# EspressoSystems/Push-CDN

Hardware: NVIDIA H100
Metric: broadcast fan-out egress GB/s (1 KiB x 2^20 subscribers per GPU, 1 topic); msgs/s and % of HBM peak alongside (higher is better)
Workload: dtype u8

## Files before the change

### push-cdn_b200/csrc/engine.cu

```cuda
#include "engine_internal.h"

namespace pcdn_detail {
thread_local std::string g_err;
int fail(int code, const std::string& msg) { g_err = msg; return code; }
}

namespace {

int flush_journal(pcdn_engine* e) {
  HostTables& t = *e->tables;
  if (!e->has_device) { t.clear_dirty(); return 0; }
  const Geometry& g = e->geo;
  bool any = !t.dirty_sub.empty() || !t.dirty_brk.empty() || !t.dirty_owner.empty() || !t.dirty_slots.empty() ||
             !t.dirty_keys.empty();
  if (!any) return 0;
  const uint32_t Ws = e->shard_W(), W = g.W;
  const bool full_keys = t.dirty_keys.size() > (size_t)g.max_keys / 16 + 64;
  const bool full_sub = t.dirty_sub.size() > t.sub.size() / 16 + 64;
  const bool full_slots = t.dirty_slots.size() > t.cuckoo.size() / 16 + 64;
  e->h_slot.clear(); e->h_kslot.clear(); e->h_kbytes.clear();
  if (!full_slots) for (uint32_t i : t.dirty_slots) e->h_slot.push_back(UpdSlot{i, t.cuckoo[i]});
  if (!full_keys) for (uint32_t k : t.dirty_keys) {
    e->h_kslot.push_back(k);
    size_t at = e->h_kbytes.size();
// ... 118 lines not shown
    for (int k = 0; k < 2; k++) {
      const int pv = sh.prev_slot[k];
      if (pv < 0 || pv == (int)si) continue;
      const ShardSlot& o = sh.slots[pv];
      if (cudaEventQuery(o.ev_done) != cudaSuccess) { cudaGetLastError(); continue; }
      const BatchStats& ps_ = *o.h_stats;
      sh.fat_only = ps_.status == 0 && ps_.n_cm == 0 && ps_.n_fat_tiles > 0 && ps_.bytes_out <= kOverlapMaxBytes;
      break;
    }
  }
  const bool fat_overlap = s.in.n_bcast > 0 && sh.fat_only;
  sh.prev_slot[1] = sh.prev_slot[0];
  sh.prev_slot[0] = (int)si;
  cudaStream_t st = sh.stream, ps = (!dp && (direct_only || fat_overlap)) ? sh.pack_stream : sh.stream, cs = sh.copy_stream;
  const bool has_direct = n_direct > 0;
  if (wait_ingest) CUDA_TRY(cudaStreamWaitEvent(st, s.ev_ingest, 0));
  s.timed = e->timing;
  s.polled = false;
  s.n_msg_errors = 0;
  if (!retry && ++s.w.stamp == 0) s.w.stamp = 1;
  if (!retry && sh.dev.pool && (s.w.stamp & 0x3FFFFFFFu) == 0) {
    s.w.stamp++;
    CUDA_TRY(cudaMemsetAsync(s.w.lb_state, 0, ((size_t)sh.dev.N / 256 + 1) * 8, st));
  }
  s.w.pool_unblock = retry ? 1u : 0u;
  s.w.batch_id = retry ? e->slots[si].batch_id : e->next_batch_id;
  const bool fused = dp && sh.dev.N <= kSmallCtrlConns && s.in.n_msgs <= kSmallCtrlMsgs &&
                     (uint64_t)s.in.n_bcast * sh.dev.nblk <= kSmallCtrlItems;
  s.spans_mapped = dp && (sh.dev.N <= 8192 || (s.in.n_bcast == 0 && s.in.n_msgs <= 4096));
  if (sh.dev.pool && !fused) s.spans_mapped = false;
  s.w.spans = s.spans_mapped ? s.d_spans_map : s.d_spans_dev;
  s.w.overflow = s.spans_mapped ? s.d_ovf_map : s.d_ovf_dev;
  const bool zero_in_kernel = fused && !devparse && !retry;
  if (s.timed) CUDA_TRY(cudaEventRecord(s.ev[0], st));
  if (retry) {
    launch_pool_retry_begin(sh.dev, s.w, st);
  } else {
    if (!zero_in_kernel) launch_batch_begin(sh.dev, s.w, s.in, has_direct, st);
    if (devparse) launch_parse(sh.dev, s.w, s.in, st);
    if (has_direct && !fused) launch_direct(sh.dev, s.w, s.in, n_direct, st);
  }
  if (s.timed) CUDA_TRY(cudaEventRecord(s.ev[1], st));
  if (fused) {
    launch_ctrl_small(sh.dev, s.w, s.in, has_direct, zero_in_kernel, s.d_stats_pub, retry, st);
    if (s.timed) { CUDA_TRY(cudaEventRecord(s.ev[2], st)); CUDA_TRY(cudaEventRecord(s.ev[3], st)); }
  } else {
    if (!retry) launch_match(sh.dev, s.w, s.in, st);
    if (s.timed) CUDA_TRY(cudaEventRecord(s.ev[2], st));
    if (!retry) launch_plan(sh.dev, s.w, s.in, st);
    launch_offsets(sh.dev, s.w, s.in, has_direct, sh.n_sms, st);
    if (s.timed) CUDA_TRY(cudaEventRecord(s.ev[3], st));
  }
  if (!s.spans_mapped) {
    CUDA_TRY(cudaEventRecord(s.ev_ctrl, st));
    CUDA_TRY(cudaStreamWaitEvent(cs, s.ev_ctrl, 0));
    CUDA_TRY(cudaMemcpyAsync(s.h_early, s.w.stats, sizeof(BatchStats), cudaMemcpyDeviceToHost, cs));
    CUDA_TRY(cudaEventRecord(s.ev_early, cs));
    if (ps != st) CUDA_TRY(cudaStreamWaitEvent(ps, s.ev_ctrl, 0));
  }
  if (s.timed) CUDA_TRY(cudaEventRecord(s.ev[4], ps));
  uint32_t pack_variant = e->cfg.pack_variant;
  if (!((pack_variant >> 8) & 15u)) pack_variant |= (fat_overlap ? 3u : 4u) << 8;
  launch_pack(sh.dev, s.w, s.in, n_direct, pack_variant, sh.n_sms, ps);
  if (s.timed) CUDA_TRY(cudaEventRecord(s.ev[5], ps));
  CUDA_TRY(cudaGetLastError());
  if (!fused) CUDA_TRY(cudaMemcpyAsync(s.h_stats, s.w.stats, sizeof(BatchStats), cudaMemcpyDeviceToHost, ps));
  CUDA_TRY(cudaEventRecord(s.ev_done, ps));
  return 0;
}

int launch_pipeline(pcdn_engine* e, uint32_t si, bool wait_ingest) {
  Slot& s = e->slots[si];
  for (Shard& sh : e->shards) {
    int rc = launch_shard_pipeline(e, sh, si, s.n_direct, s.devparse, wait_ingest);
    if (rc) return rc;
  }
  s.state = SLOT_INFLIGHT;
  s.t_launch = std::chrono::steady_clock::now();
  s.batch_id = e->next_batch_id++;
  s.counted = false;
  e->inflight.push_back(s.batch_id);
  e->open_slot = -1;
  e->stats.batches++;
  e->stats.msgs += s.n_msgs;
  return 0;
}

struct IngestRegion { const void* src; size_t dst_off; size_t bytes; bool host = false; };
int ingest_batch(pcdn_engine* e, uint32_t si, const IngestRegion* regs, int nregs, bool arena_in_place, bool wait_submit) {
  const size_t all_hi = regs[nregs - 1].dst_off + regs[nregs - 1].bytes;
  if (e->ingest == PCDN_INGEST_HOST) {
    for (Shard& sh : e->shards) {
      DeviceGuard dg(sh.device);
      ShardSlot& ss = sh.slots[si];
      CUDA_TRY(cudaStreamWaitEvent(sh.ingest_stream, ss.ev_done, 0));
      if (wait_submit) CUDA_TRY(cudaStreamWaitEvent(sh.ingest_stream, e->shards[0].ev_submit, 0));
      for (int r = 0; r < nregs; r++) {
        const IngestRegion& g = regs[r];
        if (!g.bytes || (sh.gindex == 0 && r == 0 && arena_in_place)) continue;
// ... 385 lines not shown
  CUDA_TRY(cudaMemsetAsync(d.sub, 0, (size_t)g.T * Ws * 4, sh.stream));
  CUDA_TRY(cudaMemsetAsync(d.brk, 0, (size_t)Ws * 4, sh.stream));
  CUDA_TRY(cudaMemsetAsync(d.owner_conn, 0xFF, (size_t)g.max_owners * 4, sh.stream));
  CUDA_TRY(cudaMemsetAsync(d.cuckoo, 0, (size_t)g.nbuckets * 4 * sizeof(CuckooEntry), sh.stream));
  CUDA_TRY(cudaMemsetAsync(d.keys, 0, (size_t)g.max_keys * g.key_stride, sh.stream));
  CUDA_TRY(cudaMemsetAsync(d.ptail, 0, (size_t)Ns * 4, sh.stream));
  CUDA_TRY(cudaMemsetAsync(d.used, 0, (size_t)Ns * 4, sh.stream));

  const uint32_t M = c.max_batch_msgs, MB = c.max_batch_bcast;
  const size_t cap_fat = (size_t)c.max_batch_deliveries;
  const size_t cap_thin = std::min<size_t>(c.max_batch_deliveries, (size_t)M * (kFatMin - 1));
  sh.slots.resize(c.batch_slots);
  for (ShardSlot& s : sh.slots) {
    DEV_ALLOC(s.d_arena, e->arena_cap);
    Work& w = s.w;
    DEV_ALLOC(w.B, (size_t)MB * Ws);
    DEV_ALLOC(w.wpre, (size_t)MB * Ws);
    DEV_ALLOC(w.cnt, (size_t)MB * d.nblk);
    DEV_ALLOC(w.base, (size_t)MB * d.nblk);
    DEV_ALLOC(w.done, MB);
    CUDA_TRY(cudaMemsetAsync(w.done, 0, (size_t)MB * 4, sh.stream));
    DEV_ALLOC(w.D, M);
    DEV_ALLOC(w.dconn, M);
    DEV_ALLOC(w.eb_fat, (size_t)M + 1);
    DEV_ALLOC(w.eb_thin, (size_t)M + 1);
    DEV_ALLOC(w.tbase, (size_t)M + 1);
    DEV_ALLOC(w.scan_tmp, 4 * ((size_t)M / 256 + 2));
    DEV_ALLOC(w.cls, M);
    DEV_ALLOC(w.cm_rank, (size_t)M + 1);
    DEV_ALLOC(w.cm_list, MB);
    DEV_ALLOC(w.jidx, M);
    DEV_ALLOC(w.efat, cap_fat);
    DEV_ALLOC(w.ecm, cap_fat);
    DEV_ALLOC(w.ethin, cap_thin);
    w.cap_fat = (uint32_t)std::min<size_t>(cap_fat, 0xFFFFFFFFu);
    w.cap_thin = (uint32_t)std::min<size_t>(cap_thin, 0xFFFFFFFFu);
    DEV_ALLOC(w.dcount, (size_t)Ns + 2);
    DEV_ALLOC(w.dloc, (size_t)Ns + 2);
    DEV_ALLOC(w.dtile, (size_t)Ns / 1024 + 3);
    DEV_ALLOC(w.dlist, M);
    DEV_ALLOC(w.hot_list, (size_t)M / kHotMin + 2);
    DEV_ALLOC(w.hot_bitmap, (size_t)kHotCtas * ((size_t)M / 32 + 1));
    DEV_ALLOC(w.scan_done, 1);
    CUDA_TRY(cudaMemsetAsync(w.scan_done, 0, 4, sh.stream));
    DEV_ALLOC(w.edir, M);
    DEV_ALLOC(w.dstart, (size_t)Ns + 1);
    DEV_ALLOC(w.dend, (size_t)Ns + 1);
    DEV_ALLOC(w.dstamp, (size_t)Ns + 1);
    CUDA_TRY(cudaMemsetAsync(w.dstamp, 0, ((size_t)Ns + 1) * 4, sh.stream));
    w.stamp = 0;
    DEV_ALLOC(w.batch_units, Ns);
    if (d.pool) {
      DEV_ALLOC(w.cbase, Ns);
      DEV_ALLOC(w.lb_state, (size_t)Ns / 256 + 1);
      DEV_ALLOC(w.lb_tot, (size_t)Ns / 256 + 1);
      CUDA_TRY(cudaMemsetAsync(w.lb_state, 0, ((size_t)Ns / 256 + 1) * 8, sh.stream));
    }
    w.pool_unblock = 0;
    const size_t span_entries = (size_t)2 * Ns * (d.span_runs ? 3 : 2) / 2;
    DEV_ALLOC(s.d_spans_dev, span_entries);
    DEV_ALLOC(s.d_ovf_dev, Ns);
    if (sh.direct_publish) {
      PIN_ALLOC_MAPPED(s.h_spans, s.d_spans_map, span_entries);
      PIN_ALLOC_MAPPED(s.h_overflow, s.d_ovf_map, (size_t)Ns);
    } else {
      PIN_ALLOC(s.h_spans, span_entries);
      PIN_ALLOC(s.h_overflow, g.shard_max_conns);
    }
    w.spans = s.d_spans_dev; w.overflow = s.d_ovf_dev;
    DEV_ALLOC(w.msg_status, M);
    PIN_ALLOC(s.h_msg_status, M);
    DEV_ALLOC(w.stats, 1);
    if (sh.direct_publish) PIN_ALLOC_MAPPED(s.h_stats, s.d_stats_pub, 1);
    else PIN_ALLOC(s.h_stats, 1);
    PIN_ALLOC(s.h_early, 1);
    CUDA_TRY(cudaEventCreateWithFlags(&s.ev_done, cudaEventDisableTiming));
    CUDA_TRY(cudaEventCreateWithFlags(&s.ev_ctrl, cudaEventDisableTiming));
    CUDA_TRY(cudaEventCreateWithFlags(&s.ev_early, cudaEventDisableTiming));
    CUDA_TRY(cudaEventCreateWithFlags(&s.ev_ingest, cudaEventDisableTiming));
    for (auto& ev : s.ev) CUDA_TRY(cudaEventCreate(&ev));
  }
  CUDA_TRY(cudaStreamSynchronize(sh.stream));
  return 0;
}

int init_nccl(pcdn_engine* e) {
  const char* why = "";
  e->nccl = nccl_api(&why);
  if (!e->nccl) return fail(PCDN_ENODEV, std::string("PCDN_INGEST_NCCL needs libnccl.so.2: ") + why);
  NcclUniqueId id;
  if (e->cfg.nccl_unique_id) std::memcpy(&id, e->cfg.nccl_unique_id, sizeof(id));
  else NCCL_TRY(e->nccl, e->nccl->GetUniqueId(&id));
  NCCL_TRY(e->nccl, e->nccl->GroupStart());
  for (Shard& sh : e->shards) {
    cudaSetDevice(sh.device);
    int rc = e->nccl->CommInitRank(&sh.comm, (int)e->world_shards, id, (int)sh.gindex);
    if (rc) { e->nccl->GroupEnd(); return fail(PCDN_ECUDA, std::string("ncclCommInitRank: ") + e->nccl->GetErrorString(rc)); }
  }
  NCCL_TRY(e->nccl, e->nccl->GroupEnd());
  for (Shard& sh : e->shards) {
    int n = 0;
    if (e->nccl->CommCount && e->nccl->CommCount(sh.comm, &n) == 0) sh.nccl_ranks = n;
  }
  return 0;
}

int init_device(pcdn_engine* e) {
// ... 1042 lines not shown
```

### push-cdn_b200/csrc/kernels.cu

```cuda
#include "kernels.cuh"

#include <atomic>

#include "frame_parse_core.h"

namespace pcdn {

std::atomic<unsigned long long> g_kernel_launches{0};
#define PCDN_COUNT_LAUNCH (void)g_kernel_launches.fetch_add(1, std::memory_order_relaxed)

unsigned long long kernel_launches() { return g_kernel_launches.load(std::memory_order_relaxed); }
void count_kernel_launch() { PCDN_COUNT_LAUNCH; }

__device__ __forceinline__ uint32_t lane_id() { return threadIdx.x & 31; }

__device__ __forceinline__ uint32_t warp_incl_scan(uint32_t v) {
  const uint32_t lane = lane_id();
#pragma unroll
  for (int o = 1; o < 32; o <<= 1) {
    uint32_t n = __shfl_up_sync(0xffffffffu, v, o);
    if (lane >= (uint32_t)o) v += n;
  }
  return v;
}
// ... 345 lines not shown
      const uint32_t q = (c - c_lo) >> 5, k = c & 31u;
      const uint32_t bit = event_bit(s, b, m, wd0 + q, k, e, e1);
#pragma unroll
      for (int x = 0; x < NW; x++)
        if ((uint32_t)x == q) v[x] = (v[x] & ~(1u << k)) | (bit << k);
    }
    while (e1 < ne && b.events[e1].conn == c) e1++;
    e = e1;
  }
}

__device__ __forceinline__ uint32_t match_word(const DevState& s, const BatchIn& b, uint32_t m, uint32_t wd) {
  const uint32_t toff = b.aux_off[m], tn = b.aux_len[m];
  const uint32_t fl = b.flags[m];
  uint32_t word = 0;
  if (fl & MSGF_TOPICS_U8) {
    const uint8_t* tb = b.arena + toff;
    for (uint32_t i = 0; i < tn; i++) {
      if ((fl & MSGF_PRUNE) && !topic_kept(tb, i, s.n_valid_topics)) continue;
      const uint32_t t = tb[i];
      if (t < s.T) word |= s.sub[(size_t)t * s.W + wd];
    }
  } else {
    for (uint32_t i = 0; i < tn; i++) {
      const uint32_t t = b.topics[toff + i];
      if (t < s.T) word |= s.sub[(size_t)t * s.W + wd];
    }
  }
  if (b.n_events) apply_events<1>(s, b, m, wd, &word);
  if (fl & MSGF_USERS_ONLY) word &= ~s.brk[wd];
  return word;
}
template <bool EVENTS>
__global__ void __launch_bounds__(256) k_match(DevState s, BatchIn b, Work w) {
  const uint32_t j = blockIdx.y, lane = lane_id();
  const uint32_t blk = blockIdx.x * 8 + (threadIdx.x >> 5);
  if (blk >= s.nblk) return;
  const uint32_t m = b.bcast_index[j];
  const uint32_t w0 = blk * kBlockWords + lane * 8;
  const uint32_t toff = b.aux_off[m], tn = b.aux_len[m], fl = b.flags[m];
  uint4 lo = make_uint4(0, 0, 0, 0), hi = make_uint4(0, 0, 0, 0);
  auto or_row = [&](uint32_t t) {
    if (t >= s.T) return;
    const uint4* row = reinterpret_cast<const uint4*>(s.sub + (size_t)t * s.W + w0);
    const uint4 a = row[0], c = row[1];
    lo.x |= a.x; lo.y |= a.y; lo.z |= a.z; lo.w |= a.w;
    hi.x |= c.x; hi.y |= c.y; hi.z |= c.z; hi.w |= c.w;
  };
  if (fl & MSGF_TOPICS_U8) {
    const uint8_t* tb = b.arena + toff;
    for (uint32_t i = 0; i < tn; i++) {
      if ((fl & MSGF_PRUNE) && !topic_kept(tb, i, s.n_valid_topics)) continue;
      or_row(tb[i]);
    }
  } else {
    for (uint32_t i = 0; i < tn; i++) or_row(b.topics[toff + i]);
  }
  if (EVENTS) {
    uint32_t v[8] = {lo.x, lo.y, lo.z, lo.w, hi.x, hi.y, hi.z, hi.w};
    apply_events<8>(s, b, m, w0, v);
    lo = make_uint4(v[0], v[1], v[2], v[3]); hi = make_uint4(v[4], v[5], v[6], v[7]);
  }
  if (fl & MSGF_USERS_ONLY) {
    const uint4* br = reinterpret_cast<const uint4*>(s.brk + w0);
    const uint4 a = br[0], c = br[1];
    lo.x &= ~a.x; lo.y &= ~a.y; lo.z &= ~a.z; lo.w &= ~a.w;
    hi.x &= ~c.x; hi.y &= ~c.y; hi.z &= ~c.z; hi.w &= ~c.w;
  }
  const uint32_t p0 = __popc(lo.x), p1 = p0 + __popc(lo.y), p2 = p1 + __popc(lo.z), p3 = p2 + __popc(lo.w);
  const uint32_t p4 = p3 + __popc(hi.x), p5 = p4 + __popc(hi.y), p6 = p5 + __popc(hi.z), p7 = p6 + __popc(hi.w);
  const uint32_t incl = warp_incl_scan(p7), ex = incl - p7;
  uint32_t last = 0;
  if (lane == 31) {
    w.cnt[(size_t)j * s.nblk + blk] = incl;
    __threadfence();
    last = atomicAdd(&w.done[j], 1u) == s.nblk - 1 ? 1u : 0u;
  }
  uint4* Bo = reinterpret_cast<uint4*>(w.B + (size_t)j * s.W + w0);
  Bo[0] = lo; Bo[1] = hi;
  uint4 pre;
  pre.x = ex | ((ex + p0) << 16); pre.y = (ex + p1) | ((ex + p2) << 16);
  pre.z = (ex + p3) | ((ex + p4) << 16); pre.w = (ex + p5) | ((ex + p6) << 16);
  *reinterpret_cast<uint4*>(w.wpre + (size_t)j * s.W + w0) = pre;
  if (__shfl_sync(0xffffffffu, last, 31)) {
    __threadfence();
    uint32_t carry = 0;
    for (uint32_t bb = 0; bb < s.nblk; bb += 32) {
      const uint32_t i = bb + lane;
      const uint32_t v = i < s.nblk ? __ldcg(w.cnt + (size_t)j * s.nblk + i) : 0;
      const uint32_t in = warp_incl_scan(v);
      if (i < s.nblk) w.base[(size_t)j * s.nblk + i] = carry + in - v;
      carry += __shfl_sync(0xffffffffu, in, 31);
    }
    if (lane == 0) { w.D[m] = carry; w.jidx[m] = j; w.done[j] = 0; }
  }
}
void launch_match(const DevState& s, const Work& w, const BatchIn& b, cudaStream_t st) {
  if (!b.n_bcast) return;
  dim3 grid((s.nblk + 7) / 8, b.n_bcast);
  if (b.n_events) PCDN_COUNT_LAUNCH, k_match<true><<<grid, 256, 0, st>>>(s, b, w);
  else PCDN_COUNT_LAUNCH, k_match<false><<<grid, 256, 0, st>>>(s, b, w);
}

__device__ __forceinline__ uint32_t frame_vec_bytes(uint32_t raw_len) { return (4u + raw_len + 15u) & ~15u; }
__device__ __forceinline__ uint32_t frame_units(uint32_t raw_len) { return (4u + raw_len + kUnit - 1u) / kUnit; }
__device__ __forceinline__ uint32_t rec_units(const DevState& s, uint32_t raw_len) {
  return s.shared_payload ? 1u : frame_units(raw_len);
}
__device__ __forceinline__ uint32_t tile_recipients(uint32_t frame_bytes) {
  const uint32_t chunk = min(frame_bytes, kChunkBytes);
  return max(32u, min(kTileRecipients, kFatTileBytes / chunk));
}

__device__ __forceinline__ void plan_classify(const DevState& s, const BatchIn& b, uint32_t m, uint32_t d, uint32_t* cls_out,
                                              uint32_t* tiles_out) {
  uint32_t cls = CLS_THIN, tiles = 0;
  if (d >= kFatMin) {
    const uint32_t len = b.raw_len[m];
    const bool dense = !s.shared_payload && ((uint64_t)d << kCmDenseShift) >= s.N && b.kind[m] == 4;
    if (dense && frame_units(len) * kUnit <= kCmMaxBytes) {
      cls = CLS_CM;
    } else {
      cls = CLS_FAT;
      const uint32_t nch = (frame_vec_bytes(len) + kChunkBytes - 1) / kChunkBytes;
      const uint32_t tr = tile_recipients(frame_vec_bytes(len));
      tiles = nch * ((d + tr - 1) / tr);
    }
  }
  *cls_out = cls; *tiles_out = tiles;
}

__global__ void __launch_bounds__(256) k_plan_a(DevState s, BatchIn b, Work w, uint32_t nblk) {
  __shared__ uint32_t sm[9];
  const uint32_t m = blockIdx.x * 256 + threadIdx.x;
// ... 148 lines not shown
  __shared__ uint32_t sm[NW + 1];
  __shared__ unsigned long long red[2][NW];
  __shared__ uint32_t span_base;
  if (w.stats->status) return;
  const uint32_t wd = c >> 5, lane = c & 31, lt = (1u << lane) - 1u;
  const uint32_t R = s.pool ? 0x7FFFFFFFu : s.ring_units;
  ConnCursor k;
  k.pt = s.pool ? 0u : s.ptail[c]; k.us = s.pool ? 0u : s.used[c]; k.bu = 0;
  k.s1_off = 0; k.s1_units = 0; k.s1_rec = 0; k.s2_units = 0; k.s2_rec = 0; k.ovf = 0; k.in2 = 0; k.bytes = 0;
  uint32_t dp = 0, de = 0;
  if (HAS_DIRECT) {
    if (SPARSE_BOUNDS) {
      if (w.dstamp[c] == w.stamp) { dp = w.dstart[c]; de = w.dend[c]; }
    } else {
      dp = dseg_start(w, c); de = dseg_start(w, c + 1);
      if (de - dp >= 2 && de - dp <= kHotMin) {
        for (uint32_t i = dp + 1; i < de; i++) {
          const uint32_t x = w.dlist[i];
          uint32_t j = i;
          while (j > dp && w.dlist[j - 1] > x) { w.dlist[j] = w.dlist[j - 1]; j--; }
          w.dlist[j] = x;
        }
      }
    }
  }
  const uint32_t* dmsg = w.dlist;

  auto emit_direct = [&](uint32_t m) {
    const uint32_t len = b.raw_len[m];
    const uint32_t off = alloc_record(k, rec_units(s, len), R, len);
    w.edir[m] = make_uint2(c, off);
  };

  __shared__ uint32_t m_mb[32], m_len[32], m_eb[32], m_slot[32], m_cls[32];
  for (uint32_t j0 = 0; j0 < b.n_bcast; j0 += 32) {
    const uint32_t nj = min(32u, b.n_bcast - j0);
    __syncthreads();
    if (threadIdx.x < nj) {
      const uint32_t m = b.bcast_index[j0 + threadIdx.x];
      const uint32_t cl = w.cls[m];
      m_mb[threadIdx.x] = m;
      m_len[threadIdx.x] = b.raw_len[m];
      m_cls[threadIdx.x] = cl;
      m_eb[threadIdx.x] = cl != CLS_THIN ? w.eb_fat[m] : w.eb_thin[m];
      m_slot[threadIdx.x] = b.slot_off16[m];
    }
    uint32_t Bw = 0, pre = 0;
    if (lane < nj) {
      const size_t at = (size_t)(j0 + lane) * s.W + wd;
      Bw = w.B[at];
      pre = w.base[(size_t)(j0 + lane) * s.nblk + (wd / kBlockWords)] + w.wpre[at];
    }
    __syncthreads();
    uint32_t hits = __ballot_sync(0xffffffffu, Bw != 0);
    while (hits) {
      const int i = __ffs(hits) - 1;
      hits &= hits - 1;
      const uint32_t word = __shfl_sync(0xffffffffu, Bw, i), p = __shfl_sync(0xffffffffu, pre, i);
      const uint32_t mb = m_mb[i];
      if (HAS_DIRECT) while (dp < de && dmsg[dp] < mb) { emit_direct(dmsg[dp]); dp++; }
      if ((word >> lane) & 1u) {
        const uint32_t rank = p + __popc(word & lt), len = m_len[i];
        const uint32_t off = alloc_record(k, rec_units(s, len), R, len);
        const uint32_t cl = m_cls[i];
        if (cl == CLS_CM) w.ecm[m_eb[i] + rank] = off;
        else if (cl == CLS_FAT) w.efat[m_eb[i] + rank] = make_uint2(c, off);
        else w.ethin[m_eb[i] + rank] = make_uint4(c, off, m_slot[i], len);
      }
    }
  }
  if (HAS_DIRECT) while (dp < de) { emit_direct(dmsg[dp]); dp++; }

  if (s.pool) {
    __shared__ uint32_t cta_prefix;
    uint32_t ctot;
    const uint32_t cex = cta_excl_scan<NW>(k.bu, &ctot, sm);
    if (LOOKBACK) {
      if (threadIdx.x < 32) {
        const uint32_t pre = pool_lookback(w, vb, ctot);
        if (threadIdx.x == 0) {
          cta_prefix = pre;
          if (vb == nvb - 1) pool_allocate(s, w, (unsigned long long)pre + ctot);
        }
      }
    } else if (threadIdx.x == 0) {
      cta_prefix = 0;
      w.lb_tot[vb] = ctot;
    }
    __syncthreads();
    k.s1_off = cta_prefix + cex;
    w.cbase[c] = k.s1_off;
  } else {
    s.ptail[c] = k.pt;
    s.used[c] = k.us;
  }
  w.batch_units[c] = k.bu;

  const uint32_t nsp = (k.s1_rec ? 1u : 0u) + (k.s2_rec ? 1u : 0u);
  uint32_t tot, ex;
// ... 176 lines not shown
    if (valid) {
      w.eb_fat[m] = e0; w.eb_thin[m] = e1; w.tbase[m] = e2; w.cm_rank[m] = e3; w.cls[m] = (uint8_t)cls;
      if (cls == CLS_CM) w.cm_list[e3] = m;
    }
    if (tid == 0) {
      w.stats->n_fat_entries = t0; w.stats->n_thin_entries = t1; w.stats->n_fat_tiles = t2; w.stats->tile_cursor = 0;
      w.stats->n_cm = t3; w.stats->cm_cursor = 0;
      if (t0 > w.cap_fat || t1 > w.cap_thin) w.stats->status = 1;
      const uint32_t n = b.n_msgs;
      w.eb_fat[n] = t0; w.eb_thin[n] = t1; w.tbase[n] = t2; w.cm_rank[n] = t3;
    }
  }
  cluster_sync_all();

  for (uint32_t c0 = 0; c0 < s.N; c0 += 8192)
    offsets_body<HAS_DIRECT, 1024, true, true>(s, b, w, s.N, c0 + rank * 1024 + tid, c0 / 1024 + rank, s.N / 1024);

  if (publish) {
    cluster_sync_all();
    if (rank == 0 && tid < sizeof(BatchStats) / 4)
      reinterpret_cast<uint32_t*>(publish)[tid] = __ldcg(reinterpret_cast<const uint32_t*>(w.stats) + tid);
  }
}
void launch_ctrl_small(const DevState& s, const Work& w, const BatchIn& b, bool has_direct, bool zero_stats,
                       BatchStats* publish, bool offsets_only, cudaStream_t st) {
  if (has_direct) PCDN_COUNT_LAUNCH, k_ctrl_small<true><<<8, 1024, 0, st>>>(s, b, w, zero_stats ? 1 : 0, publish, offsets_only ? 1 : 0);
  else PCDN_COUNT_LAUNCH, k_ctrl_small<false><<<8, 1024, 0, st>>>(s, b, w, zero_stats ? 1 : 0, publish, offsets_only ? 1 : 0);
}

__global__ void k_pool_retry_begin(BatchStats* bs) {
  bs->status = 0;
  bs->n_deliveries = 0; bs->bytes_out = 0;
  bs->n_spans = 0; bs->n_runs = 0; bs->n_overflow = 0;
  bs->tile_cursor = 0; bs->cm_cursor = 0;
}
void launch_pool_retry_begin(const DevState& s, const Work& w, cudaStream_t st) {
  cudaMemsetAsync(w.lb_state, 0, ((size_t)s.N / 256 + 1) * 8, st);
  PCDN_COUNT_LAUNCH, k_pool_retry_begin<<<1, 1, 0, st>>>(w.stats);
}

__device__ __forceinline__ uint8_t* conn_out(const DevState& s, const Work& w, uint32_t conn, uint32_t pool_base) {
  return s.pool ? s.rings + ((size_t)pool_base + w.cbase[conn]) * kUnit : s.rings + (size_t)conn * s.ring_bytes;
}

__device__ __forceinline__ void pack_fat_phase(const DevState& s, const BatchIn& b, const Work& w, uint8_t* buf,
                                               uint64_t* barp) {
  uint64_t& bar = *barp;
  __shared__ uint32_t t_info[8];
  const uint32_t tid = threadIdx.x;
  const uint32_t ntiles = w.stats->n_fat_tiles;
  if (ntiles == 0) return;
  const uint32_t pool_base = w.stats->pool_base;
  uint32_t phase = 0;
  uint32_t staged_m = 0xFFFFFFFFu, staged_k = 0xFFFFFFFFu;

  for (;;) {
    if (tid == 0) {
      const uint32_t t = atomicAdd(&w.stats->tile_cursor, 1u);
      t_info[0] = t;
      if (t < ntiles) {
        uint32_t lo = 0, hi = b.n_msgs;
        while (hi - lo > 1) { uint32_t mid = (lo + hi) >> 1; if (w.tbase[mid] <= t) lo = mid; else hi = mid; }
        const uint32_t m = lo, ltile = t - w.tbase[m], d = w.D[m];
        const uint32_t fb = frame_vec_bytes(b.raw_len[m]);
        const uint32_t tr = tile_recipients(fb);
        const uint32_t ngrp = (d + tr - 1) / tr;
        const uint32_t ch = ltile / ngrp, grp = ltile % ngrp;
// ... 37 lines not shown
  bulk_wait_read0();
}

__device__ __forceinline__ void pack_cm_phase(const DevState& s, const BatchIn& b, const Work& w, uint8_t* buf,
                                              uint64_t* barp) {
  uint64_t& bar = *barp;
  __shared__ uint32_t g_m[kCmGroup], g_j[kCmGroup], g_soff[kCmGroup], g_units[kCmGroup], g_eb[kCmGroup];
  __shared__ uint32_t t_info[4];
  const uint32_t tid = threadIdx.x, lane = tid & 31, warp = tid >> 5;
  if (w.stats->status) return;
  const uint32_t ncm = w.stats->n_cm;
  if (ncm == 0) return;
  const uint32_t pool_base = w.stats->pool_base;
  const uint32_t ngroups = (ncm + kCmGroup - 1) / kCmGroup;
  const uint32_t tpg = s.W / kCmTileWords;
  const uint32_t ntiles = ngroups * tpg;
  uint32_t phase = 0;
  uint32_t staged_g = 0xFFFFFFFFu;

  for (;;) {
    if (tid == 0) {
      const uint32_t t = atomicAdd(&w.stats->cm_cursor, 1u);
      t_info[0] = t;
      if (t < ntiles) {
        const uint32_t g = t / tpg;
        const uint32_t gcount = min(kCmGroup, ncm - g * kCmGroup);
        t_info[1] = g; t_info[2] = gcount;
        t_info[3] = g != staged_g ? 1u : 0u;
        staged_g = g;
      }
    }
    __syncthreads();
    if (t_info[0] >= ntiles) break;
    const uint32_t gcount = t_info[2];
    if (t_info[3]) {
      bulk_wait_read0();
      __syncthreads();
      if (tid == 0) {
        const uint32_t g = t_info[1];
        uint32_t soff = 0, total = 0;
        for (uint32_t i = 0; i < gcount; i++) {
          const uint32_t m = w.cm_list[g * kCmGroup + i];
          const uint32_t len = b.raw_len[m];
          g_m[i] = m; g_j[i] = w.jidx[m]; g_soff[i] = soff; g_units[i] = frame_units(len); g_eb[i] = w.eb_fat[m];
          soff += frame_units(len) * kUnit;
          total += frame_vec_bytes(len);
        }
        mbar_arrive_expect_tx(&bar, total);
        for (uint32_t i = 0; i < gcount; i++)
          bulk_g2s(buf + g_soff[i], b.arena + (size_t)b.slot_off16[g_m[i]] * 16, frame_vec_bytes(b.raw_len[g_m[i]]), &bar);
      }
      __syncthreads();
      mbar_wait(&bar, phase);
      phase ^= 1;
      if (tid < gcount) {
        *reinterpret_cast<uint32_t*>(buf + g_soff[tid]) = bswap32(b.raw_len[g_m[tid]]);
        fence_proxy_async_smem();
      }
      __syncthreads();
    }
    const uint32_t wt = t_info[0] % tpg;
    for (uint32_t wi = warp; wi < kCmTileWords; wi += 8) {
      const uint32_t wd = wt * kCmTileWords + wi;
      const uint32_t myword = lane < gcount ? w.B[(size_t)g_j[lane] * s.W + wd] : 0u;
      const uint32_t any = __reduce_or_sync(0xffffffffu, myword);
      if (!any) continue;
      uint32_t offs[kCmGroup];
#pragma unroll
      for (int i = 0; i < (int)kCmGroup; i++) {
        const uint32_t wordi = __shfl_sync(0xffffffffu, myword, i);
        offs[i] = kOffInvalid;
        if ((uint32_t)i < gcount && ((wordi >> lane) & 1u)) {
          const uint32_t j = g_j[i];
          const uint32_t idx = g_eb[i] + w.base[(size_t)j * s.nblk + wd / kBlockWords] + w.wpre[(size_t)j * s.W + wd] +
                               __popc(wordi & ((1u << lane) - 1u));
          offs[i] = w.ecm[idx];
        }
      }
      uint8_t* ring = conn_out(s, w, wd * 32 + lane, pool_base);
      uint32_t run_o = kOffInvalid, run_units = 0, run_s = 0;
#pragma unroll
      for (int i = 0; i < (int)kCmGroup; i++) {
        const uint32_t o = offs[i];
        if (o != kOffInvalid && run_o != kOffInvalid && o == run_o + run_units) {
          run_units += g_units[i];
        } else {
          if (run_o != kOffInvalid) bulk_s2g(ring + (size_t)run_o * kUnit, buf + run_s, run_units * kUnit);
          run_o = o; run_s = g_soff[i]; run_units = (o != kOffInvalid) ? g_units[i] : 0;
        }
      }
      if (run_o != kOffInvalid) bulk_s2g(ring + (size_t)run_o * kUnit, buf + run_s, run_units * kUnit);
    }
    bulk_commit();
    __syncthreads();
  }
  bulk_wait_read0();
}

__device__ __forceinline__ void copy_record(const uint4* __restrict__ src, uint4* __restrict__ dst, uint32_t raw_len, uint32_t lane) {
  const uint32_t nvec = (4u + raw_len + 15u) >> 4;
  const uint32_t hdr = bswap32(raw_len);
  for (uint32_t v = lane; v < nvec; v += 128) {
    uint4 x0, x1, x2, x3;
    const bool p1 = v + 32 < nvec, p2 = v + 64 < nvec, p3 = v + 96 < nvec;
    x0 = ld_nc16(src + v);
    if (p1) x1 = ld_nc16(src + v + 32);
    if (p2) x2 = ld_nc16(src + v + 64);
    if (p3) x3 = ld_nc16(src + v + 96);
    if (v == 0) x0.x = hdr;
// ... 4 lines not shown
  }
}
__device__ __forceinline__ void pack_thin_phase(const DevState& s, const BatchIn& b, const Work& w) {
  const uint32_t n = w.stats->n_thin_entries;
  const uint32_t pool_base = w.stats->pool_base;
  const uint32_t lane = lane_id();
  const uint32_t gw = (blockIdx.x * blockDim.x + threadIdx.x) >> 5, nw = (gridDim.x * blockDim.x) >> 5;
  for (uint32_t e = gw; e < n; e += nw) {
    const uint4 ent = w.ethin[e];
    if (ent.y == kOffInvalid) continue;
    copy_record(reinterpret_cast<const uint4*>(b.arena + (size_t)ent.z * 16),
                reinterpret_cast<uint4*>(conn_out(s, w, ent.x, pool_base) + (size_t)ent.y * kUnit), ent.w, lane);
  }
}
__device__ __forceinline__ void pack_direct_phase(const DevState& s, const BatchIn& b, const Work& w) {
  const uint32_t n = b.n_msgs;
  const uint32_t pool_base = w.stats->pool_base;
  const uint32_t lane = lane_id();
  const uint32_t gw = (blockIdx.x * blockDim.x + threadIdx.x) >> 5, nw = (gridDim.x * blockDim.x) >> 5;
  uint2 ent = make_uint2(0, kOffInvalid);
  uint32_t so = 0, len = 0;
  if (gw < n) { ent = w.edir[gw]; so = b.slot_off16[gw]; len = b.raw_len[gw]; }
  for (uint32_t m = gw; m < n; m += nw) {
    const uint2 cur = ent;
    const uint32_t cso = so, clen = len;
    const uint32_t nx = m + nw;
    if (nx < n) { ent = w.edir[nx]; so = b.slot_off16[nx]; len = b.raw_len[nx]; }
    if (cur.y == kOffInvalid) continue;
    copy_record(reinterpret_cast<const uint4*>(b.arena + (size_t)cso * 16),
                reinterpret_cast<uint4*>(conn_out(s, w, cur.x, pool_base) + (size_t)cur.y * kUnit), clen, lane);
  }
}

__global__ void __launch_bounds__(256) k_pack(DevState s, BatchIn b, Work w, int do_direct) {
  __shared__ __align__(128) uint8_t buf[kCmGroup * kCmMaxBytes];
  __shared__ __align__(8) uint64_t bars[2];
  if (w.stats->status) return;
  if (threadIdx.x == 0) {
    mbar_init(&bars[0], 1);
    mbar_init(&bars[1], 1);
    asm volatile("fence.mbarrier_init.release.cluster;" ::: "memory");
  }
  __syncthreads();
  pack_cm_phase(s, b, w, buf, &bars[0]);
  __syncthreads();
  pack_fat_phase(s, b, w, buf, &bars[1]);
  pack_thin_phase(s, b, w);
  if (do_direct) pack_direct_phase(s, b, w);
}
__global__ void __launch_bounds__(256, 8) k_pack_direct(DevState s, BatchIn b, Work w) {
  if (w.stats->status) return;
  pack_direct_phase(s, b, w);
}

__device__ __forceinline__ void st_ref_record(uint8_t* dst, uint32_t raw_len, uint32_t slot_off16, unsigned long long batch_id) {
  const unsigned long long off = (unsigned long long)slot_off16 * 16u + 4u;
  st_stream16(dst, make_uint4(0xFFFFFFFFu, bswap32(raw_len), (uint32_t)off, (uint32_t)(off >> 32)));
  st_stream16(dst + 16, make_uint4((uint32_t)batch_id, (uint32_t)(batch_id >> 32), 0u, 0u));
}
__global__ void __launch_bounds__(256) k_pack_ref(DevState s, BatchIn b, Work w, int do_direct) {
  if (w.stats->status) return;
  const uint32_t nfat = w.stats->n_fat_entries, nthin = w.stats->n_thin_entries;
  const uint64_t nft = (uint64_t)nfat + nthin, total = nft + (do_direct ? b.n_msgs : 0u);
  const uint32_t pool_base = w.stats->pool_base;
  const unsigned long long bid = w.batch_id;
  const uint64_t stride = (uint64_t)gridDim.x * blockDim.x;
  for (uint64_t i = (uint64_t)blockIdx.x * blockDim.x + threadIdx.x; i < total; i += stride) {
    uint32_t conn, off, m = 0, slot = 0, len = 0;
    bool thin = false;
    if (i < nfat) {
      const uint32_t e = (uint32_t)i;
      uint32_t lo = 0, hi = b.n_msgs;
      while (hi - lo > 1) { const uint32_t mid = (lo + hi) >> 1; if (w.eb_fat[mid] <= e) lo = mid; else hi = mid; }
      const uint2 ent = w.efat[e];
      conn = ent.x; off = ent.y; m = lo;
    } else if (i < nft) {
      const uint4 ent = w.ethin[i - nfat];
      conn = ent.x; off = ent.y; slot = ent.z; len = ent.w; thin = true;
    } else {
      m = (uint32_t)(i - nft);
      const uint2 ent = w.edir[m];
      conn = ent.x; off = ent.y;
    }
    if (off == kOffInvalid) continue;
    if (!thin) { slot = b.slot_off16[m]; len = b.raw_len[m]; }
    st_ref_record(conn_out(s, w, conn, pool_base) + (size_t)off * kUnit, len, slot, bid);
  }
}

void launch_pack(const DevState& s, const Work& w, const BatchIn& b, uint32_t n_direct, uint32_t pack_variant, int n_sms, cudaStream_t st) {
  if (s.shared_payload) {
    if (b.n_bcast || n_direct) PCDN_COUNT_LAUNCH, k_pack_ref<<<(uint32_t)n_sms * 8, 256, 0, st>>>(s, b, w, n_direct ? 1 : 0);
    return;
  }
  const bool direct_separate = n_direct >= kThinSeparateMin;
  const uint32_t ctas_per_sm = ((pack_variant >> 8) & 15u) ? ((pack_variant >> 8) & 15u) : 3;
  const uint32_t grid = (uint32_t)n_sms * ctas_per_sm;
  const int do_direct = (n_direct && !direct_separate) ? 1 : 0;
  if (b.n_bcast || do_direct)
    PCDN_COUNT_LAUNCH, k_pack<<<grid, 256, 0, st>>>(s, b, w, do_direct);
  const uint32_t dctas = ((pack_variant >> 12) & 15u) ? ((pack_variant >> 12) & 15u) : 8u;
  if (direct_separate) PCDN_COUNT_LAUNCH, k_pack_direct<<<(uint32_t)n_sms * dctas, 256, 0, st>>>(s, b, w);
}

__global__ void __launch_bounds__(256) k_release(DevState s, const uint32_t* __restrict__ batch_units,
                                                 const BatchStats* __restrict__ stats) {
  if (stats->status) return;
  const uint32_t i = blockIdx.x * blockDim.x + threadIdx.x;
  if (i * 4 < s.N) {
    const uint4 u = reinterpret_cast<const uint4*>(batch_units)[i];
    if (u.x | u.y | u.z | u.w) {
      uint4* p = reinterpret_cast<uint4*>(s.used) + i;
      uint4 v = *p;
      v.x -= u.x; v.y -= u.y; v.z -= u.z; v.w -= u.w;
      *p = v;
    }
  }
}
__global__ void k_pool_release(PoolState* p, const BatchStats* __restrict__ stats) {
  if (stats->status) return;
  p->used -= stats->pool_units + stats->pool_skip;
  p->tail = stats->pool_base + stats->pool_units;
  if (p->used == 0) { p->head = 0; p->tail = 0; }
}
__global__ void k_pool_init(PoolState* p) { p->head = 0; p->tail = 0; p->used = 0; p->blocked = 0; }
void launch_pool_init(const DevState& s, cudaStream_t st) {
  if (s.pool) PCDN_COUNT_LAUNCH, k_pool_init<<<1, 1, 0, st>>>(s.pool_state);
}
void launch_release(const DevState& s, const uint32_t* batch_units, const BatchStats* stats, cudaStream_t st) {
  if (s.pool) { PCDN_COUNT_LAUNCH, k_pool_release<<<1, 1, 0, st>>>(s.pool_state, stats); return; }
  PCDN_COUNT_LAUNCH, k_release<<<(s.N / 4 + 255) / 256, 256, 0, st>>>(s, batch_units, stats);
}

}
```

### push-cdn_b200/csrc/kernels.cuh

```cuda
#pragma once
#include <cuda_runtime.h>
#include <stdint.h>

#include "hash.h"

namespace pcdn {

constexpr uint32_t kUnit = 32;
constexpr uint32_t kOffInvalid = 0xFFFFFFFFu;
constexpr uint32_t kConnNone = 0xFFFFFFFFu;
constexpr uint32_t kFatMin = 32;
constexpr uint32_t kChunkBytes = 16384;
constexpr uint32_t kTileRecipients = 1024;
constexpr uint32_t kFatTileBytes = 131072;
constexpr uint32_t kBlockWords = 256;
constexpr uint32_t kCmGroup = 8;
constexpr uint32_t kCmMaxBytes = 4096;
constexpr uint32_t kSmallCtrlConns = 65536;
constexpr uint32_t kSmallCtrlMsgs = 256;
constexpr uint32_t kSmallCtrlItems = 256;
constexpr uint32_t kThinSeparateMin = 2048;
constexpr uint32_t kHotMin = 32;
constexpr uint32_t kHotCtas = 32;
constexpr uint32_t kCmTileWords = 16;
constexpr uint32_t kCmDenseShift = 4;
enum : uint8_t { CLS_THIN = 0, CLS_FAT = 1, CLS_CM = 2 };
enum : uint8_t {
  MSGF_USERS_ONLY = 1,
  MSGF_DEVPARSE = 2,
  MSGF_TOPICS_U8 = 4,
  MSGF_PRUNE = 8
};
constexpr int8_t kErrParse = -7, kErrPrune = -8;

struct DevState {
  uint32_t* sub;
  uint32_t* brk;
  uint32_t* owner_conn;
  CuckooEntry* cuckoo;
  uint8_t* keys;
  uint32_t* ptail;
  uint32_t* used;
// ... 26 lines not shown
  uint32_t n_msgs, n_bcast;
  const uint8_t* arena;
  const uint8_t* kind;
  const uint8_t* flags;
  const uint32_t* slot_off16;
  const uint32_t* raw_len;
  const uint32_t* aux_off;
  const uint32_t* aux_len;
  const uint16_t* topics;
  const uint32_t* bcast_index;
  uint32_t n_events;
  const SubEvent* events;
  const uint16_t* ev_topics;
};

struct BatchStats {
  unsigned long long n_deliveries;
  unsigned long long bytes_out;
  uint32_t n_spans;
  uint32_t n_overflow;
  uint32_t n_direct_dropped;
  uint32_t status;
  uint32_t n_fat_entries;
  uint32_t n_thin_entries;
  uint32_t n_fat_tiles;
  uint32_t tile_cursor;
  uint32_t n_cm;
  uint32_t cm_cursor;
  uint32_t n_hot;
  uint32_t n_runs;
  uint32_t pool_base;
  uint32_t pool_units;
  uint32_t pool_skip;
  uint32_t reserved;
};

struct PoolState { uint32_t head, tail, used, blocked; };

struct Span { uint32_t conn, ring_off, len, n_records; };
struct SpanRun { uint32_t conn0, n_conns, ring_off, len, n_records, off_stride; };

struct Work {
  uint32_t* B;
  uint16_t* wpre;
  uint32_t* cnt;
  uint32_t* base;
  uint32_t* done;
  uint32_t* D;
  uint32_t* dconn;
  uint32_t* eb_fat;
  uint32_t* eb_thin;
  uint32_t* tbase;
  uint32_t* scan_tmp;
  uint8_t* cls;
  uint32_t* cm_rank;
  uint32_t* cm_list;
  uint32_t* jidx;
  uint2* efat;
  uint32_t* ecm;
  uint4* ethin;
  uint32_t cap_fat, cap_thin;
  uint32_t* dcount;
  uint32_t* dloc;
  uint32_t* dtile;
  uint32_t* dlist;
  uint32_t* hot_list;
  uint32_t* hot_bitmap;
  uint32_t* scan_done;
  uint2* edir;
  uint32_t* dstart;
  uint32_t* dend;
  uint32_t* dstamp;
  uint32_t stamp;
  uint32_t* cbase;
  unsigned long long* lb_state;
  uint32_t* lb_tot;
  uint32_t pool_unblock;
  unsigned long long batch_id;
  uint32_t* batch_units;
  Span* spans;
  uint32_t* overflow;
  int8_t* msg_status;
  BatchStats* stats;
};

struct Upd32 { uint32_t arr, idx, val; };
struct UpdSlot { uint32_t slot; CuckooEntry e; };

void launch_apply_updates(const DevState& s, const Upd32* u32, uint32_t n32, const UpdSlot* us,
                          uint32_t nslot, const uint32_t* key_slots, const uint8_t* key_bytes,
                          uint32_t nkeys, cudaStream_t st);
void launch_batch_begin(const DevState& s, const Work& w, const BatchIn& b, bool has_direct, cudaStream_t st);
void launch_parse(const DevState& s, const Work& w, const BatchIn& b, cudaStream_t st);
void launch_direct(const DevState& s, const Work& w, const BatchIn& b, uint32_t n_direct, cudaStream_t st);
void launch_match(const DevState& s, const Work& w, const BatchIn& b, cudaStream_t st);
void launch_plan(const DevState& s, const Work& w, const BatchIn& b, cudaStream_t st);
void launch_offsets(const DevState& s, const Work& w, const BatchIn& b, bool has_direct, int n_sms, cudaStream_t st);
void launch_ctrl_small(const DevState& s, const Work& w, const BatchIn& b, bool has_direct, bool zero_stats,
                       BatchStats* publish, bool offsets_only, cudaStream_t st);
void launch_pool_retry_begin(const DevState& s, const Work& w, cudaStream_t st);
void launch_pack(const DevState& s, const Work& w, const BatchIn& b, uint32_t n_direct, uint32_t pack_variant, int n_sms, cudaStream_t st);
void launch_release(const DevState& s, const uint32_t* batch_units, const BatchStats* stats, cudaStream_t st);
void launch_pool_init(const DevState& s, cudaStream_t st);
unsigned long long kernel_launches();
void count_kernel_launch();

}
```

Before: 2928.

## Fold stats zeroing into match, publish stats from pack, and run-encode CM offsets

Three separate changes. Stats zeroing moves into the match kernel, which removes the batch_begin launch for pure-broadcast batches. The last pack CTA now writes the stats into mapped host memory, replacing the device-to-host memcpy. The CM offset entries are also run-length encoded per connection and group, so the pack phase can rebuild consecutive offsets instead of gathering ecm per message. In exchange this adds a cmrun buffer, per-thread shared-memory state in the offsets kernel, and a grid-wide atomic plus system fence at the end of pack.

```diff
diff --git a/push-cdn_b200/csrc/engine.cu b/push-cdn_b200/csrc/engine.cu
--- a/push-cdn_b200/csrc/engine.cu
+++ b/push-cdn_b200/csrc/engine.cu
@@ -174,11 +174,12 @@
   s.w.spans = s.spans_mapped ? s.d_spans_map : s.d_spans_dev;
   s.w.overflow = s.spans_mapped ? s.d_ovf_map : s.d_ovf_dev;
   const bool zero_in_kernel = fused && !devparse && !retry;
+  const bool zero_in_match = !fused && !devparse && !retry && !has_direct && s.in.n_bcast > 0;
   if (s.timed) CUDA_TRY(cudaEventRecord(s.ev[0], st));
   if (retry) {
     launch_pool_retry_begin(sh.dev, s.w, st);
   } else {
-    if (!zero_in_kernel) launch_batch_begin(sh.dev, s.w, s.in, has_direct, st);
+    if (!zero_in_kernel && !zero_in_match) launch_batch_begin(sh.dev, s.w, s.in, has_direct, st);
     if (devparse) launch_parse(sh.dev, s.w, s.in, st);
     if (has_direct && !fused) launch_direct(sh.dev, s.w, s.in, n_direct, st);
   }
@@ -187,7 +188,7 @@
     launch_ctrl_small(sh.dev, s.w, s.in, has_direct, zero_in_kernel, s.d_stats_pub, retry, st);
     if (s.timed) { CUDA_TRY(cudaEventRecord(s.ev[2], st)); CUDA_TRY(cudaEventRecord(s.ev[3], st)); }
   } else {
-    if (!retry) launch_match(sh.dev, s.w, s.in, st);
+    if (!retry) launch_match(sh.dev, s.w, s.in, zero_in_match ? s.w.stats : nullptr, st);
     if (s.timed) CUDA_TRY(cudaEventRecord(s.ev[2], st));
     if (!retry) launch_plan(sh.dev, s.w, s.in, st);
     launch_offsets(sh.dev, s.w, s.in, has_direct, sh.n_sms, st);
@@ -203,10 +204,10 @@
   if (s.timed) CUDA_TRY(cudaEventRecord(s.ev[4], ps));
   uint32_t pack_variant = e->cfg.pack_variant;
   if (!((pack_variant >> 8) & 15u)) pack_variant |= (fat_overlap ? 3u : 4u) << 8;
-  launch_pack(sh.dev, s.w, s.in, n_direct, pack_variant, sh.n_sms, ps);
+  const bool published = launch_pack(sh.dev, s.w, s.in, n_direct, pack_variant, sh.n_sms, fused ? nullptr : s.d_stats_pub, ps);
   if (s.timed) CUDA_TRY(cudaEventRecord(s.ev[5], ps));
   CUDA_TRY(cudaGetLastError());
-  if (!fused) CUDA_TRY(cudaMemcpyAsync(s.h_stats, s.w.stats, sizeof(BatchStats), cudaMemcpyDeviceToHost, ps));
+  if (!fused && !published) CUDA_TRY(cudaMemcpyAsync(s.h_stats, s.w.stats, sizeof(BatchStats), cudaMemcpyDeviceToHost, ps));
   CUDA_TRY(cudaEventRecord(s.ev_done, ps));
   return 0;
 }
@@ -658,6 +659,7 @@
     DEV_ALLOC(w.jidx, M);
     DEV_ALLOC(w.efat, cap_fat);
     DEV_ALLOC(w.ecm, cap_fat);
+    DEV_ALLOC(w.cmrun, std::min<size_t>(((size_t)MB + kCmGroup - 1) / kCmGroup * Ns, 2 * cap_fat + Ns));
     DEV_ALLOC(w.ethin, cap_thin);
     w.cap_fat = (uint32_t)std::min<size_t>(cap_fat, 0xFFFFFFFFu);
     w.cap_thin = (uint32_t)std::min<size_t>(cap_thin, 0xFFFFFFFFu);
@@ -697,8 +699,7 @@
     DEV_ALLOC(w.msg_status, M);
     PIN_ALLOC(s.h_msg_status, M);
     DEV_ALLOC(w.stats, 1);
-    if (sh.direct_publish) PIN_ALLOC_MAPPED(s.h_stats, s.d_stats_pub, 1);
-    else PIN_ALLOC(s.h_stats, 1);
+    PIN_ALLOC_MAPPED(s.h_stats, s.d_stats_pub, 1);
     PIN_ALLOC(s.h_early, 1);
     CUDA_TRY(cudaEventCreateWithFlags(&s.ev_done, cudaEventDisableTiming));
     CUDA_TRY(cudaEventCreateWithFlags(&s.ev_ctrl, cudaEventDisableTiming));
diff --git a/push-cdn_b200/csrc/kernels.cu b/push-cdn_b200/csrc/kernels.cu
--- a/push-cdn_b200/csrc/kernels.cu
+++ b/push-cdn_b200/csrc/kernels.cu
@@ -401,7 +401,8 @@
   return word;
 }
 template <bool EVENTS>
-__global__ void __launch_bounds__(256) k_match(DevState s, BatchIn b, Work w) {
+__global__ void __launch_bounds__(256) k_match(DevState s, BatchIn b, Work w, BatchStats* zero) {
+  if (zero && blockIdx.x == 0 && blockIdx.y == 0 && threadIdx.x < sizeof(BatchStats) / 4) reinterpret_cast<uint32_t*>(zero)[threadIdx.x] = 0;
   const uint32_t j = blockIdx.y, lane = lane_id();
   const uint32_t blk = blockIdx.x * 8 + (threadIdx.x >> 5);
   if (blk >= s.nblk) return;
@@ -464,11 +465,11 @@
     if (lane == 0) { w.D[m] = carry; w.jidx[m] = j; w.done[j] = 0; }
   }
 }
-void launch_match(const DevState& s, const Work& w, const BatchIn& b, cudaStream_t st) {
+void launch_match(const DevState& s, const Work& w, const BatchIn& b, BatchStats* zero, cudaStream_t st) {
   if (!b.n_bcast) return;
   dim3 grid((s.nblk + 7) / 8, b.n_bcast);
-  if (b.n_events) PCDN_COUNT_LAUNCH, k_match<true><<<grid, 256, 0, st>>>(s, b, w);
-  else PCDN_COUNT_LAUNCH, k_match<false><<<grid, 256, 0, st>>>(s, b, w);
+  if (b.n_events) PCDN_COUNT_LAUNCH, k_match<true><<<grid, 256, 0, st>>>(s, b, w, zero);
+  else PCDN_COUNT_LAUNCH, k_match<false><<<grid, 256, 0, st>>>(s, b, w, zero);
 }
 
 __device__ __forceinline__ uint32_t frame_vec_bytes(uint32_t raw_len) { return (4u + raw_len + 15u) & ~15u; }
@@ -683,7 +684,13 @@
     w.edir[m] = make_uint2(c, off);
   };
 
-  __shared__ uint32_t m_mb[32], m_len[32], m_eb[32], m_slot[32], m_cls[32];
+  __shared__ uint32_t cm_last_[NT], cm_first_[NT], cm_start_[NT], cm_next_[NT];
+  uint32_t& cm_start = cm_start_[threadIdx.x];
+  uint32_t& cm_next = cm_next_[threadIdx.x];
+  cm_last_[threadIdx.x] = kOffInvalid;
+
+  __shared__ uint32_t m_mb[32], m_len[32], m_eb[32], m_slot[32], m_cls[32], m_cmr[32];
+  __shared__ uint32_t* m_run[32];
   for (uint32_t j0 = 0; j0 < b.n_bcast; j0 += 32) {
     const uint32_t nj = min(32u, b.n_bcast - j0);
     __syncthreads();
@@ -693,6 +700,11 @@
       m_mb[threadIdx.x] = m;
       m_len[threadIdx.x] = b.raw_len[m];
       m_cls[threadIdx.x] = cl;
+      if (cl == CLS_CM) {
+        const uint32_t r = w.cm_rank[m];
+        m_cmr[threadIdx.x] = r;
+        m_run[threadIdx.x] = w.cmrun + (size_t)(r / kCmGroup) * s.N;
+      }
       m_eb[threadIdx.x] = cl != CLS_THIN ? w.eb_fat[m] : w.eb_thin[m];
       m_slot[threadIdx.x] = b.slot_off16[m];
     }
@@ -712,10 +724,25 @@
       if (HAS_DIRECT) while (dp < de && dmsg[dp] < mb) { emit_direct(dmsg[dp]); dp++; }
       if ((word >> lane) & 1u) {
         const uint32_t rank = p + __popc(word & lt), len = m_len[i];
-        const uint32_t off = alloc_record(k, rec_units(s, len), R, len);
+        const uint32_t u = rec_units(s, len);
+        const uint32_t off = alloc_record(k, u, R, len);
         const uint32_t cl = m_cls[i];
-        if (cl == CLS_CM) w.ecm[m_eb[i] + rank] = off;
-        else if (cl == CLS_FAT) w.efat[m_eb[i] + rank] = make_uint2(c, off);
+        if (cl == CLS_CM) {
+          uint32_t* row = m_run[i];
+          const uint32_t r = m_cmr[i];
+          if ((r ^ cm_last_[threadIdx.x]) >= kCmGroup) {
+            cm_start = off != kOffInvalid ? off : kCmBroken | (r & (kCmGroup - 1));
+            cm_first_[threadIdx.x] = m_eb[i] + rank;
+            row[c] = cm_start;
+          } else if (cm_start < kCmBroken && off != cm_next) {
+            w.ecm[cm_first_[threadIdx.x]] = cm_start;
+            cm_start = kCmBroken | (r & (kCmGroup - 1));
+            row[c] = cm_start;
+          }
+          if (cm_start >= kCmBroken) w.ecm[m_eb[i] + rank] = off;
+          cm_last_[threadIdx.x] = r;
+          cm_next = off + u;
+        } else if (cl == CLS_FAT) w.efat[m_eb[i] + rank] = make_uint2(c, off);
         else w.ethin[m_eb[i] + rank] = make_uint4(c, off, m_slot[i], len);
       }
     }
@@ -958,7 +985,7 @@
   bs->status = 0;
   bs->n_deliveries = 0; bs->bytes_out = 0;
   bs->n_spans = 0; bs->n_runs = 0; bs->n_overflow = 0;
-  bs->tile_cursor = 0; bs->cm_cursor = 0;
+  bs->tile_cursor = 0; bs->cm_cursor = 0; bs->ctas_done = 0;
 }
 void launch_pool_retry_begin(const DevState& s, const Work& w, cudaStream_t st) {
   cudaMemsetAsync(w.lb_state, 0, ((size_t)s.N / 256 + 1) * 8, st);
@@ -1062,7 +1089,7 @@
     }
     __syncthreads();
     if (t_info[0] >= ntiles) break;
-    const uint32_t gcount = t_info[2];
+    const uint32_t grp = t_info[1], gcount = t_info[2];
     if (t_info[3]) {
       bulk_wait_read0();
       __syncthreads();
@@ -1095,16 +1122,28 @@
       const uint32_t myword = lane < gcount ? w.B[(size_t)g_j[lane] * s.W + wd] : 0u;
       const uint32_t any = __reduce_or_sync(0xffffffffu, myword);
       if (!any) continue;
+      uint32_t mine = 0;
+#pragma unroll
+      for (int i = 0; i < (int)kCmGroup; i++)
+        mine |= ((__shfl_sync(0xffffffffu, myword, i) >> lane) & 1u) << i;
+      mine &= (1u << gcount) - 1u;
       uint32_t offs[kCmGroup];
+      const uint32_t run = mine ? w.cmrun[(size_t)grp * s.N + wd * 32 + lane] : kOffInvalid;
+      const uint32_t brk = run >= kCmBroken ? run - kCmBroken : kCmGroup;
+      uint32_t cur = run;
+      bool first = true;
 #pragma unroll
       for (int i = 0; i < (int)kCmGroup; i++) {
-        const uint32_t wordi = __shfl_sync(0xffffffffu, myword, i);
         offs[i] = kOffInvalid;
-        if ((uint32_t)i < gcount && ((wordi >> lane) & 1u)) {
-          const uint32_t j = g_j[i];
-          const uint32_t idx = g_eb[i] + w.base[(size_t)j * s.nblk + wd / kBlockWords] + w.wpre[(size_t)j * s.W + wd] +
-                               __popc(wordi & ((1u << lane) - 1u));
-          offs[i] = w.ecm[idx];
+        if ((mine >> i) & 1u) {
+          if (brk < kCmGroup && (first || (uint32_t)i >= brk)) {
+            const uint32_t j = g_j[i];
+            const size_t at = (size_t)j * s.W + wd;
+            cur = w.ecm[g_eb[i] + w.base[(size_t)j * s.nblk + wd / kBlockWords] + w.wpre[at] + __popc(w.B[at] & ((1u << lane) - 1u))];
+          }
+          offs[i] = cur;
+          first = false;
+          if (cur != kOffInvalid) cur += g_units[i];
         }
       }
       uint8_t* ring = conn_out(s, w, wd * 32 + lane, pool_base);
@@ -1175,25 +1214,43 @@
   }
 }
 
-__global__ void __launch_bounds__(256) k_pack(DevState s, BatchIn b, Work w, int do_direct) {
+__device__ __forceinline__ void publish_if_last(const Work& w, BatchStats* publish) {
+  if (!publish) return;
+  __shared__ uint32_t last;
+  __syncthreads();
+  if (threadIdx.x == 0) {
+    __threadfence();
+    last = atomicAdd(&w.stats->ctas_done, 1u) == gridDim.x - 1 ? 1u : 0u;
+  }
+  __syncthreads();
+  if (last && threadIdx.x < sizeof(BatchStats) / 4) {
+    __threadfence();
+    reinterpret_cast<volatile uint32_t*>(publish)[threadIdx.x] = __ldcg(reinterpret_cast<const uint32_t*>(w.stats) + threadIdx.x);
+    __threadfence_system();
+  }
+}
+
+__global__ void __launch_bounds__(256) k_pack(DevState s, BatchIn b, Work w, int do_direct, BatchStats* publish) {
   __shared__ __align__(128) uint8_t buf[kCmGroup * kCmMaxBytes];
   __shared__ __align__(8) uint64_t bars[2];
-  if (w.stats->status) return;
-  if (threadIdx.x == 0) {
-    mbar_init(&bars[0], 1);
-    mbar_init(&bars[1], 1);
-    asm volatile("fence.mbarrier_init.release.cluster;" ::: "memory");
-  }
-  __syncthreads();
-  pack_cm_phase(s, b, w, buf, &bars[0]);
-  __syncthreads();
-  pack_fat_phase(s, b, w, buf, &bars[1]);
-  pack_thin_phase(s, b, w);
-  if (do_direct) pack_direct_phase(s, b, w);
-}
-__global__ void __launch_bounds__(256, 8) k_pack_direct(DevState s, BatchIn b, Work w) {
-  if (w.stats->status) return;
-  pack_direct_phase(s, b, w);
+  if (!w.stats->status) {
+    if (threadIdx.x == 0) {
+      mbar_init(&bars[0], 1);
+      mbar_init(&bars[1], 1);
+      asm volatile("fence.mbarrier_init.release.cluster;" ::: "memory");
+    }
+    __syncthreads();
+    pack_cm_phase(s, b, w, buf, &bars[0]);
+    __syncthreads();
+    pack_fat_phase(s, b, w, buf, &bars[1]);
+    pack_thin_phase(s, b, w);
+    if (do_direct) pack_direct_phase(s, b, w);
+  }
+  publish_if_last(w, publish);
+}
+__global__ void __launch_bounds__(256, 8) k_pack_direct(DevState s, BatchIn b, Work w, BatchStats* publish) {
+  if (!w.stats->status) pack_direct_phase(s, b, w);
+  publish_if_last(w, publish);
 }
 
 __device__ __forceinline__ void st_ref_record(uint8_t* dst, uint32_t raw_len, uint32_t slot_off16, unsigned long long batch_id) {
@@ -1201,8 +1258,8 @@
   st_stream16(dst, make_uint4(0xFFFFFFFFu, bswap32(raw_len), (uint32_t)off, (uint32_t)(off >> 32)));
   st_stream16(dst + 16, make_uint4((uint32_t)batch_id, (uint32_t)(batch_id >> 32), 0u, 0u));
 }
-__global__ void __launch_bounds__(256) k_pack_ref(DevState s, BatchIn b, Work w, int do_direct) {
-  if (w.stats->status) return;
+__global__ void __launch_bounds__(256) k_pack_ref(DevState s, BatchIn b, Work w, int do_direct, BatchStats* publish) {
+  if (w.stats->status) { publish_if_last(w, publish); return; }
   const uint32_t nfat = w.stats->n_fat_entries, nthin = w.stats->n_thin_entries;
   const uint64_t nft = (uint64_t)nfat + nthin, total = nft + (do_direct ? b.n_msgs : 0u);
   const uint32_t pool_base = w.stats->pool_base;
@@ -1229,21 +1286,25 @@
     if (!thin) { slot = b.slot_off16[m]; len = b.raw_len[m]; }
     st_ref_record(conn_out(s, w, conn, pool_base) + (size_t)off * kUnit, len, slot, bid);
   }
-}
-
-void launch_pack(const DevState& s, const Work& w, const BatchIn& b, uint32_t n_direct, uint32_t pack_variant, int n_sms, cudaStream_t st) {
+  publish_if_last(w, publish);
+}
+
+bool launch_pack(const DevState& s, const Work& w, const BatchIn& b, uint32_t n_direct, uint32_t pack_variant, int n_sms,
+                 BatchStats* publish, cudaStream_t st) {
   if (s.shared_payload) {
-    if (b.n_bcast || n_direct) PCDN_COUNT_LAUNCH, k_pack_ref<<<(uint32_t)n_sms * 8, 256, 0, st>>>(s, b, w, n_direct ? 1 : 0);
-    return;
+    if (!b.n_bcast && !n_direct) return false;
+    PCDN_COUNT_LAUNCH, k_pack_ref<<<(uint32_t)n_sms * 8, 256, 0, st>>>(s, b, w, n_direct ? 1 : 0, publish);
+    return true;
   }
   const bool direct_separate = n_direct >= kThinSeparateMin;
   const uint32_t ctas_per_sm = ((pack_variant >> 8) & 15u) ? ((pack_variant >> 8) & 15u) : 3;
   const uint32_t grid = (uint32_t)n_sms * ctas_per_sm;
   const int do_direct = (n_direct && !direct_separate) ? 1 : 0;
   if (b.n_bcast || do_direct)
-    PCDN_COUNT_LAUNCH, k_pack<<<grid, 256, 0, st>>>(s, b, w, do_direct);
+    PCDN_COUNT_LAUNCH, k_pack<<<grid, 256, 0, st>>>(s, b, w, do_direct, direct_separate ? nullptr : publish);
   const uint32_t dctas = ((pack_variant >> 12) & 15u) ? ((pack_variant >> 12) & 15u) : 8u;
-  if (direct_separate) PCDN_COUNT_LAUNCH, k_pack_direct<<<(uint32_t)n_sms * dctas, 256, 0, st>>>(s, b, w);
+  if (direct_separate) PCDN_COUNT_LAUNCH, k_pack_direct<<<(uint32_t)n_sms * dctas, 256, 0, st>>>(s, b, w, publish);
+  return direct_separate || b.n_bcast || do_direct;
 }
 
 __global__ void __launch_bounds__(256) k_release(DevState s, const uint32_t* __restrict__ batch_units,
diff --git a/push-cdn_b200/csrc/kernels.cuh b/push-cdn_b200/csrc/kernels.cuh
--- a/push-cdn_b200/csrc/kernels.cuh
+++ b/push-cdn_b200/csrc/kernels.cuh
@@ -8,6 +8,7 @@
 
 constexpr uint32_t kUnit = 32;
 constexpr uint32_t kOffInvalid = 0xFFFFFFFFu;
+constexpr uint32_t kCmBroken = 0xFFFFFFF0u;
 constexpr uint32_t kConnNone = 0xFFFFFFFFu;
 constexpr uint32_t kFatMin = 32;
 constexpr uint32_t kChunkBytes = 16384;
@@ -100,7 +101,7 @@
   uint32_t pool_base;
   uint32_t pool_units;
   uint32_t pool_skip;
-  uint32_t reserved;
+  uint32_t ctas_done;
 };
 
 struct PoolState { uint32_t head, tail, used, blocked; };
@@ -126,6 +127,7 @@
   uint32_t* jidx;
   uint2* efat;
   uint32_t* ecm;
+  uint32_t* cmrun;
   uint4* ethin;
   uint32_t cap_fat, cap_thin;
   uint32_t* dcount;
@@ -161,13 +163,14 @@
 void launch_batch_begin(const DevState& s, const Work& w, const BatchIn& b, bool has_direct, cudaStream_t st);
 void launch_parse(const DevState& s, const Work& w, const BatchIn& b, cudaStream_t st);
 void launch_direct(const DevState& s, const Work& w, const BatchIn& b, uint32_t n_direct, cudaStream_t st);
-void launch_match(const DevState& s, const Work& w, const BatchIn& b, cudaStream_t st);
+void launch_match(const DevState& s, const Work& w, const BatchIn& b, BatchStats* zero, cudaStream_t st);
 void launch_plan(const DevState& s, const Work& w, const BatchIn& b, cudaStream_t st);
 void launch_offsets(const DevState& s, const Work& w, const BatchIn& b, bool has_direct, int n_sms, cudaStream_t st);
 void launch_ctrl_small(const DevState& s, const Work& w, const BatchIn& b, bool has_direct, bool zero_stats,
                        BatchStats* publish, bool offsets_only, cudaStream_t st);
 void launch_pool_retry_begin(const DevState& s, const Work& w, cudaStream_t st);
-void launch_pack(const DevState& s, const Work& w, const BatchIn& b, uint32_t n_direct, uint32_t pack_variant, int n_sms, cudaStream_t st);
+bool launch_pack(const DevState& s, const Work& w, const BatchIn& b, uint32_t n_direct, uint32_t pack_variant, int n_sms,
+                 BatchStats* publish, cudaStream_t st);
 void launch_release(const DevState& s, const uint32_t* batch_units, const BatchStats* stats, cudaStream_t st);
 void launch_pool_init(const DevState& s, cudaStream_t st);
 unsigned long long kernel_launches();
```

Result: faster. 3036 (median of 6 runs) (+3.7%).
